# DreamWaterFound/self_commit_ORB-SLAM2

Measured on AMD Instinct MI355X. Metric: frames/s ORB extract+match (1000 feat, 640x480), higher is better.
Workload: dtype u8; 1 GPU; batch of 256 synthetic 640x480 frames per GPU (8 distinct resident batches per step, one launch set per batch), ORB extract (1000 feat, 8 levels, FAST 20/7) + brute-force Hamming SearchByBoW of consecutive frames; batch_per_gpu=256, streams=3, width=640, height=480, nfeatures=1000, parallelism=frames sharded, 1 rank(s), no data-path collective

## Files before the change

self_commit_orb-slam2_amd/csrc/orbx_kernels.hip:

```cpp
#include <algorithm>
#include "orbx_internal.h"

namespace {

struct OdTables {
    float pat[256][4];
    uint32_t disc[64][4];
};
constexpr int8_t kPattern[1024] = {
#include "orb_pattern.inc"
};
constexpr int kUmax[16] = {15, 15, 15, 15, 14, 14, 14, 13, 13, 12, 11, 10, 9, 8, 6, 3};
constexpr OdTables make_od_tables()
{
    OdTables t{};
    for (int i = 0; i < 256; i++) {
        t.pat[i][0] = (float)kPattern[4 * i]; t.pat[i][2] = (float)kPattern[4 * i + 1];
        t.pat[i][1] = (float)kPattern[4 * i + 2]; t.pat[i][3] = (float)kPattern[4 * i + 3];
    }
    for (int ml = 0; ml < 64; ml++)
        for (int j = 0; j < 4; j++) {
            const int mr = ml >> 1, mh = ml & 1;
            uint32_t m = 0u;
            if (mr < 31) {
// ... 746 lines not shown
        ncand = nToExpand + sh_misc[3];
        const bool finish = newN >= N || newN == prev;
        for (int j = tid; j < M; j += BT) {
            const int nd = (int)lab[j];
            if (!sel[nd]) { lab[j] = nmap[nd][0]; continue; }
            const uint32_t p = pts[j];
            const int nl = nmap[nd][ot_quadrant(p, box[cur][nd])];
            lab[j] = (uint32_t)nl;
            if (!finish && cnt[nxt][nl] > 1) atomicAdd(&qc[nxt][nl][ot_quadrant(p, box[nxt][nl])], 1u);
        }
        __syncthreads();
        if (tid == 0) { sh_misc[2] = 0; sh_misc[3] = 0; }
        nn = newN;
        cur = nxt;
        if (finish) break;
        if (!careful && nn + nToExpand * 3 > N) careful = true;
    }

    {
        uint32_t *best = &qc[cur ^ 1][0][0];
        OrbxLevelKp *out = lvlKp + (size_t)f * g->kpPerFrame + lv.kpBase;
        if (nn > lv.kpCap) { if (tid == 0) { atomicOr(stat, ORBX_DEV_ERR_KPCAP); atomicOr(statAll, ORBX_DEV_ERR_KPCAP); } nn = lv.kpCap; }
        __syncthreads();
        for (int i = tid; i < NODECAP; i += BT) best[i] = 0u;
        __syncthreads();
        for (int j = tid; j < M; j += BT) {
            const uint32_t nd = lab[j];
            if (nd < (uint32_t)NODECAP) atomicMax(&best[nd], (pts[j] & 0xff000000u) | (0x00ffffffu - (uint32_t)j));
        }
        __syncthreads();
        for (int i = tid; i < nn; i += BT) {
            const uint32_t b = pts[0x00ffffffu - (best[i] & 0x00ffffffu)];
            OrbxLevelKp kp;
            kp.x = (uint16_t)((b & 0xfff) + ORBX_BORDER); kp.y = (uint16_t)(((b >> 12) & 0xfff) + ORBX_BORDER);
            kp.score = (uint8_t)(b >> 24); kp.pad[0] = kp.pad[1] = kp.pad[2] = 0; kp.angle = 0.f; kp.ca = 1.f; kp.sb = 0.f;
            out[i] = kp;
        }
        if (tid == 0) lvlCnt[f * g->nlevels + l] = nn;
    }
}

__device__ __forceinline__ void host_pyramid_copy(const OrbxGeom *__restrict__ g, const OrbxCombMember *__restrict__ comb, const uint8_t *__restrict__ engPyr, int f, int chunk, int nchunks)
{
    uint4 *dst = (uint4 *)comb[f].hostPyr;
    if (!dst) return;
    const uint4 *src = (const uint4 *)(engPyr + (size_t)f * g->pyrBytes);
    const size_t n = g->pyrBytes >> 4, bt = blockDim.x, stride = (size_t)nchunks * bt;
    for (size_t i = (size_t)chunk * bt + threadIdx.x; i < n; i += stride) dst[i] = src[i];
}

template <int NODECAP>
__global__ __launch_bounds__(256) void k_octree(const OrbxGeom *__restrict__ g, const int *__restrict__ cellCount, const uint32_t *__restrict__ cellSlots,
                                                const uint8_t *__restrict__ binTab, uint32_t *__restrict__ ptBuf, uint32_t *__restrict__ labBuf,
                                                OrbxLevelKp *__restrict__ lvlKp, int *__restrict__ lvlCnt, int *__restrict__ status,
                                                const OrbxCombMember *__restrict__ comb, const uint8_t *__restrict__ engPyr, int *__restrict__ outBase)
{
    XCD_REMAP_XY(l, f);
    if (l >= g->nlevels) {
        host_pyramid_copy(g, comb, engPyr, f, l - g->nlevels, (int)gridDim.x - g->nlevels);
        return;
    }
    octree_body<NODECAP, 256>(g, cellCount, cellSlots, binTab, ptBuf, labBuf, lvlKp, lvlCnt, status, l, f, (int)gridDim.y);
    if (outBase && threadIdx.x == 0) {
        const int n = lvlCnt[f * g->nlevels + l];
        for (int j = l + 1; j < g->nlevels; j++) atomicAdd(&outBase[f * g->nlevels + j], n);
    }
}

__device__ __forceinline__ float sinf_poly_d(double x, double x2, int n, bool neg)
{
    const double c0 = 0x1p0, c1 = -0x1.ffffffd0c621cp-2, c2 = 0x1.55553e1068f19p-5, c3 = -0x1.6c087e89a359dp-10, c4 = 0x1.99343027bf8c3p-16;
    const double s1 = -0x1.555545995a603p-3, s2 = 0x1.1107605230bc4p-7, s3 = -0x1.994eb3774cf24p-13;
    if ((n & 1) == 0) {
        double x3 = x * x2, t1 = s2 + x2 * s3, x7 = x3 * x2, s = x + x3 * s1;
        return (float)(s + x7 * t1);
    } else {
        double k0 = neg ? -c0 : c0, k1 = neg ? -c1 : c1, k2 = neg ? -c2 : c2, k3 = neg ? -c3 : c3, k4 = neg ? -c4 : c4;
        double x4 = x2 * x2, u2 = k3 + x2 * k4, u1 = k0 + x2 * k1, x6 = x4 * x2, c = u1 + x4 * k2;
        return (float)(c + x6 * u2);
    }
}

__device__ __forceinline__ void sincosf_glibc(float y, float &sn, float &cs)
{
    double x = y;
    const uint32_t top = (__float_as_uint(y) >> 20) & 0x7ff;
    if (top < ((0x3f490fdbu >> 20) & 0x7ff)) {
        double x2 = x * x;
        if (top < ((0x39800000u >> 20) & 0x7ff)) { sn = y; cs = 1.0f; return; }
        sn = sinf_poly_d(x, x2, 0, false);
        cs = sinf_poly_d(x, x2, 1, false);
        return;
    }
    double r = x * 0x1.45F306DC9C883p+23;
    int n = ((int)r + 0x800000) >> 24;
    x = x - n * 0x1.921FB54442D18p0;
    const double sgn = ((n & 3) == 1 || (n & 3) == 2) ? -1.0 : 1.0;
    const bool neg = (n & 2) != 0;
    sn = sinf_poly_d(x * sgn, x * x, n, neg);
    cs = sinf_poly_d(x * sgn, x * x, n ^ 1, neg);
}

__device__ __forceinline__ float fast_atan2_deg(float y, float x)
{
    const float scale = (float)(180.0 / 3.14159265358979323846);
    const float p1 = 0.9997878412794807f * scale, p3 = -0.3258083974640975f * scale, p5 = 0.1555786518463281f * scale,
                p7 = -0.04432655554792128f * scale;
    float ax = fabsf(x), ay = fabsf(y), a, c, c2;
    if (ax >= ay) {
        c = ay / (ax + 2.220446049250313e-16f);
        c2 = c * c;
        a = (((p7 * c2 + p5) * c2 + p3) * c2 + p1) * c;
    } else {
        c = ax / (ay + 2.220446049250313e-16f);
        c2 = c * c;
        a = 90.f - (((p7 * c2 + p5) * c2 + p3) * c2 + p1) * c;
    }
    if (x < 0) a = 180.f - a;
    if (y < 0) a = 360.f - a;
    return a;
}

#define BT_W 64
#define BT_H 32
#define BT_P 80
#define BT_IH (BT_H + 6)

__device__ __forceinline__ int reflect101(int p, int len)
{
    if (p < 0) p = -p;
    if (p >= len) p = 2 * len - 2 - p;
    return p;
}

template <bool CLAMP>
__device__ __forceinline__ void blur_rows8(const OrbxGeom *__restrict__ g, const uint32_t *__restrict__ win, const int pitchW, uint32_t outw[8])
{
    const uint32_t k0 = g->taps[0], k1 = g->taps[1], k2 = g->taps[2], k3 = g->taps[3], k4 = g->taps[4], k5 = g->taps[5], k6 = g->taps[6];
    const uint32_t A0 = (k0 << 8) | (k1 << 16) | (k2 << 24), A1 = k3 | (k4 << 8) | (k5 << 16) | (k6 << 24);
    const uint32_t B0 = (k0 << 16) | (k1 << 24), B1 = k2 | (k3 << 8) | (k4 << 16) | (k5 << 24), B2 = k6;
    const uint32_t C0 = k0 << 24, C1 = k1 | (k2 << 8) | (k3 << 16) | (k4 << 24), C2 = k5 | (k6 << 8);
    const uint32_t D1 = k0 | (k1 << 8) | (k2 << 16) | (k3 << 24), D2 = k4 | (k5 << 8) | (k6 << 16);
    uint32_t hp[4][7];
#pragma unroll
    for (int m = 0; m < 7; m++) {
        uint32_t o[2][4];
#pragma unroll
        for (int s = 0; s < 2; s++) {
            const uint32_t *pw = win + (2 * m + s) * pitchW;
            const uint32_t w0 = pw[0], w1 = pw[1], w2 = pw[2];
            o[s][0] = __builtin_amdgcn_udot4(w1, A1, __builtin_amdgcn_udot4(w0, A0, 0u, false), false);
            o[s][1] = __builtin_amdgcn_udot4(w2, B2, __builtin_amdgcn_udot4(w1, B1, __builtin_amdgcn_udot4(w0, B0, 0u, false), false), false);
            o[s][2] = __builtin_amdgcn_udot4(w2, C2, __builtin_amdgcn_udot4(w1, C1, __builtin_amdgcn_udot4(w0, C0, 0u, false), false), false);
            o[s][3] = __builtin_amdgcn_udot4(w2, D2, __builtin_amdgcn_udot4(w1, D1, 0u, false), false);
        }
#pragma unroll
        for (int j = 0; j < 4; j++) hp[j][m] = o[0][j] | (o[1][j] << 16);
    }
    const uint32_t E0 = k0 | (k1 << 16), E1 = k2 | (k3 << 16), E2 = k4 | (k5 << 16), E3 = k6;
    const uint32_t O0 = k0 << 16, O1 = k1 | (k2 << 16), O2 = k3 | (k4 << 16), O3 = k5 | (k6 << 16);
#pragma unroll
    for (int q = 0; q < 8; q++) outw[q] = 0;
#pragma unroll
    for (int j = 0; j < 4; j++) {
        const uint32_t selo = j == 0 ? 0x03020106u : j == 1 ? 0x03020600u : j == 2 ? 0x03060100u : 0x06020100u;
#pragma unroll
        for (int q = 0; q < 8; q++) {
            const int t = q >> 1;
            const uint32_t sum = (q & 1) ? udot2(hp[j][t + 3], O3, udot2(hp[j][t + 2], O2, udot2(hp[j][t + 1], O1, udot2(hp[j][t], O0, 32768u))))
                                         : udot2(hp[j][t + 3], E3, udot2(hp[j][t + 2], E2, udot2(hp[j][t + 1], E1, udot2(hp[j][t], E0, 32768u))));
            if (CLAMP) outw[q] |= min(sum >> 16, 255u) << (8 * j);
            else outw[q] = __builtin_amdgcn_perm(sum, outw[q], selo);
        }
    }
}

template <bool CLAMP>
__device__ __forceinline__ void blur_body(const OrbxGeom *__restrict__ g, const uint8_t *__restrict__ img0, int img0Stride, size_t img0FramePitch,
                                          const uint8_t *__restrict__ pyr, uint8_t *__restrict__ blur, const int bx, const int f, uint32_t *__restrict__ in, const int lane,
                                          const bool store)
{
    int bases[ORBX_MAX_LEVELS];
    const int nl = g->nlevels;
    for (int i = 0; i < nl; i++) bases[i] = g->lv[i].blurTileBase;
    const int l = find_level(bases, nl, bx);
    const OrbxLevel &lv = g->lv[l];
    const int t = bx - lv.blurTileBase;
    const int X0 = (t % lv.blurTilesX) * BT_W, Y0 = (t / lv.blurTilesX) * BT_H;
    const int w = lv.w, h = lv.h;
    int pitch;
    const uint8_t *src = level_ptr(g, l, f, img0, img0Stride, img0FramePitch, pyr, pitch);
#pragma unroll
    for (int it = 0; it < 3; it++) {
        const int item = lane + 64 * it;
        if (item < BT_IH * 5) {
            const int r = (item * 205) >> 10, c = item - 5 * r;
            int y = reflect101(Y0 - 3 + r, h);
            y = min(max(y, 0), h - 1);
            const int x = X0 - 8 + 16 * c;
            const uint8_t *row = src + (size_t)y * pitch;
            uint4 v;
            if (x >= 0 && x + 15 < w) __builtin_memcpy(&v, row + x, 16);
            else {
                const int xs = min(max(x, 0), w - 16), d = x - xs;
                uint4 sv;
                __builtin_memcpy(&sv, row + xs, 16);
                if (d < 0) v = make_uint4(0u, 0u, sv.x, sv.y);
                else {
                    const uint32_t sw[8] = {sv.x, sv.y, sv.z, sv.w, 0u, 0u, 0u, 0u};
                    const int q = min(d >> 2, 4), bsh = d & 3;
                    uint32_t o[4];
#pragma unroll
                    for (int k = 0; k < 4; k++) {
                        uint32_t lo = 0u, hi = 0u;
#pragma unroll
                        for (int t = 0; t < 8; t++) { lo = (k + q == t) ? sw[t] : lo; hi = (k + q + 1 == t) ? sw[t] : hi; }
                        o[k] = bsh == 0 ? lo : bsh == 1 ? __builtin_amdgcn_alignbyte(hi, lo, 1) : bsh == 2 ? __builtin_amdgcn_alignbyte(hi, lo, 2) : __builtin_amdgcn_alignbyte(hi, lo, 3);
                    }
                    v = make_uint4(o[0], o[1], o[2], o[3]);
                }
            }
            *(uint4 *)(in + r * (BT_P / 4) + 4 * c) = v;
        }
    }
    __syncthreads();
    if (X0 == 0 || X0 + BT_W + 3 > w) {
        uint8_t *inb = (uint8_t *)in;
        if (lane < BT_IH) {
            uint8_t *rowb = inb + lane * BT_P;
            if (X0 == 0) { rowb[7] = rowb[9]; rowb[6] = rowb[10]; rowb[5] = rowb[11]; }
#pragma unroll
            for (int k = 0; k < 3; k++) {
                const int xo = w + k - X0 + 8, xi = w - 2 - k - X0 + 8;
                if (xo >= 0 && xo < BT_P && xi >= 0 && xi < BT_P) rowb[xo] = rowb[xi];
            }
        }
    }
    __syncthreads();
    const int gq = lane & 15, rg = lane >> 4;
    const int x = X0 + 4 * gq;
    if (!store || x >= w || Y0 + 8 * rg >= h) return;
    uint32_t outw[8];
    blur_rows8<CLAMP>(g, in + 8 * rg * (BT_P / 4) + gq + 1, BT_P / 4, outw);
    uint8_t *dst = blur + (size_t)f * g->pyrBytes + lv.off;
#pragma unroll
    for (int q = 0; q < 8; q++) {
        const int y = Y0 + 8 * rg + q;
        if (y >= h) break;
        *(uint32_t *)(dst + (size_t)y * lv.pitch + x) = outw[q];
    }
}

template <bool CLAMP>
__global__ __launch_bounds__(64) void k_blur(const OrbxGeom *__restrict__ g, const uint8_t *__restrict__ img0, int img0Stride, size_t img0FramePitch,
                                             const uint8_t *__restrict__ pyr, uint8_t *__restrict__ blur, const int *__restrict__ lvlCnt, int *__restrict__ outBase)
{
    __shared__ __attribute__((aligned(16))) uint32_t in[BT_IH * (BT_P / 4)];
    XCD_REMAP_XY(bx, f);
    if (bx == 0 && threadIdx.x == 0 && outBase) {
        int run = 0;
        for (int i = 0; i < g->nlevels; i++) { outBase[f * g->nlevels + i] = run; run += lvlCnt[f * g->nlevels + i]; }
    }
    blur_body<CLAMP>(g, img0, img0Stride, img0FramePitch, pyr, blur, bx, f, in, (int)threadIdx.x, true);
}

#define PB_THREADS 256
#define PB_ORG 16
#define PB_STAGE 4
__device__ __forceinline__ int pb_div(int item, uint32_t dv) { return (int)(__umul24((uint32_t)item, dv & 0xfffffu) >> (dv >> 20)); }
__device__ __forceinline__ uint32_t pb_mulhi24(uint32_t a, uint32_t b) { return __umulhi(a, b); }
template <bool EDGE>
__device__ __forceinline__ void pb_stage(uint8_t *__restrict__ bb, const uint8_t *__restrict__ src, const int sp, const int readable, const int w, const int h, const int P,
                                         const int s0, const int nr, const uint32_t divNc, const int tid)
{
    const int nc = (w + 15) >> 4, items = nr * nc;
    for (int i0 = 0; i0 < items; i0 += PB_THREADS * PB_STAGE) {
        uint4 v[PB_STAGE];
        int dOff[PB_STAGE];
#pragma unroll
        for (int k = 0; k < PB_STAGE; k++) {
            const int item = i0 + tid + k * PB_THREADS, it = min(item, items - 1);
            const int r = pb_div(it, divNc), c = it - (int)__umul24((uint32_t)r, (uint32_t)nc);
            int y = s0 - 3 + r;
            if (EDGE) {
                y = reflect101(y, h);
                y = min(max(y, 0), h - 1);
            }
            const uint8_t *row = src + (size_t)y * sp;
            const int x = 16 * c;
            if (x + 16 <= readable) __builtin_memcpy(&v[k], row + x, 16);
            else {
                uint32_t t[4] = {0u, 0u, 0u, 0u};
                for (int j = 0; x + j < w; j++) t[j >> 2] |= (uint32_t)row[x + j] << (8 * (j & 3));
                v[k] = make_uint4(t[0], t[1], t[2], t[3]);
            }
            dOff[k] = item < items ? (int)__umul24((uint32_t)r, (uint32_t)P) + PB_ORG + x : -1;
        }
#pragma unroll
        for (int k = 0; k < PB_STAGE; k++)
            if (dOff[k] >= 0) *(uint4 *)(bb + dOff[k]) = v[k];
    }
}

template <bool CLAMP>
__global__ __launch_bounds__(PB_THREADS) void k_pyr_band(const OrbxGeom *__restrict__ g, const int l, const uint8_t *__restrict__ img0, int img0Stride, size_t img0FramePitch,
                                                         const int readable, uint8_t *__restrict__ pyr, uint8_t *__restrict__ blur, const uint32_t *__restrict__ rsTab,
                                                         int *__restrict__ outBase)
{
    extern __shared__ __attribute__((aligned(16))) uint32_t band[];
    uint8_t *bb = (uint8_t *)band;
    XCD_REMAP_XY(b, f);
    const int nl = g->nlevels, tid = (int)threadIdx.x;
    if (l == 0 && b == 0 && tid < nl && outBase) outBase[f * nl + tid] = 0;
    const OrbxLevel &lv = g->lv[l];
    const int w = lv.w, h = lv.h, P = lv.bandPitch;
    const int s0 = b * lv.bandH, s1 = min(s0 + lv.bandH, h);
    const int nr = ((s1 - s0 + 7) & ~7) + 6;
    int sp;
    const uint8_t *src = level_ptr(g, l, f, img0, img0Stride, img0FramePitch, pyr, sp);
    if (s0 >= 3 && s0 - 3 + nr <= h) pb_stage<false>(bb, src, sp, readable, w, h, P, s0, nr, lv.bandDivNc, tid);
    else pb_stage<true>(bb, src, sp, readable, w, h, P, s0, nr, lv.bandDivNc, tid);
    __syncthreads();
    for (int r = tid; r < nr; r += PB_THREADS) {
        uint8_t *rowb = bb + r * P + PB_ORG;
        rowb[-1] = rowb[1]; rowb[-2] = rowb[2]; rowb[-3] = rowb[3];
#pragma unroll
        for (int k = 0; k < 3; k++) rowb[w + k] = rowb[w - 2 - k];
    }
    __syncthreads();
    {
        const int G4 = (w + 3) >> 2, items = G4 * ((s1 - s0 + 7) >> 3), PW = P >> 2;
        const uint32_t pitch = (uint32_t)lv.pitch;
        const bool full = ((s1 - s0) & 7) == 0;
        uint8_t *dst = blur + (size_t)f * g->pyrBytes + lv.off;
        for (int item = tid; item < items; item += PB_THREADS) {
            const int rgi = pb_div(item, lv.bandDivG4), gx = item - (int)__umul24((uint32_t)rgi, (uint32_t)G4);
            uint32_t outw[8];
            blur_rows8<CLAMP>(g, band + (int)__umul24((uint32_t)(8 * rgi), (uint32_t)PW) + gx + PB_ORG / 4 - 1, PW, outw);
            uint32_t o = (uint32_t)(s0 + 8 * rgi) * pitch + 4u * (uint32_t)gx;
            if (full) {
#pragma unroll
                for (int q = 0; q < 8; q++, o += pitch) *(uint32_t *)(dst + o) = outw[q];
            } else {
#pragma unroll
                for (int q = 0; q < 8; q++, o += pitch) {
                    if (s0 + 8 * rgi + q >= s1) break;
                    *(uint32_t *)(dst + o) = outw[q];
                }
            }
        }
    }
    if (l + 1 >= nl) return;
    const OrbxLevel &ln = g->lv[l + 1];
    const int d0 = (int)rsTab[lv.bandOff + b], d1 = (int)rsTab[lv.bandOff + b + 1];
    const int Gd = (ln.w + 3) >> 2, items = Gd * ((d1 - d0 + 7) >> 3);
    const uint32_t dpitch = (uint32_t)ln.pitch;
    const uint2 *rt = (const uint2 *)(rsTab + ln.rsRowOff);
    const uint32_t *ctab = rsTab + ln.rsColOff;
    uint8_t *dstBase = pyr + (size_t)f * g->pyrBytes + ln.off;
    const uint8_t *lrow0 = bb + PB_ORG - (s0 - 3) * P;
    for (int item = tid; item < items; item += PB_THREADS) {
        const int ch = pb_div(item, ln.bandDivG4), cg = item - (int)__umul24((uint32_t)ch, (uint32_t)Gd);
        const uint32_t *ct = ctab + 12u * (uint32_t)cg;
        const uint4 c0 = *(const uint4 *)ct, c1 = *(const uint4 *)(ct + 4), c2 = *(const uint4 *)(ct + 8);
        const int sx0 = (int)c0.x, sxa = sx0 & ~3;
        const uint32_t mis = (uint32_t)(sx0 & 3);
        const bool wide = (int)c0.y <= 7;
        const uint32_t sel[4] = {c0.z, c0.w, c1.x, c1.y}, coef[4] = {c1.z, c1.w, c2.x, c2.y};
        auto hpass = [&](int y, uint32_t hv[4]) {
            const uint8_t *row = lrow0 + (int)__umul24((uint32_t)y, (uint32_t)P);
            if (wide) {
                const uint32_t *p = (const uint32_t *)(row + sxa);
                const uint32_t a0 = p[0], a1 = p[1], a2 = p[2];
                const uint32_t v0 = __builtin_amdgcn_alignbyte(a1, a0, mis), v1 = __builtin_amdgcn_alignbyte(a2, a1, mis);
#pragma unroll
                for (int k = 0; k < 4; k++) hv[k] = udot2(__builtin_amdgcn_perm(v1, v0, sel[k]), coef[k], 0u) & 0x00fffff0u;
            } else {
                const uint8_t *S = row + sx0;
#pragma unroll
                for (int k = 0; k < 4; k++) {
                    const int off = (int)((c2.z >> (8 * k)) & 0xffu), off1 = (int)((c2.w >> (8 * k)) & 0xffu);
                    hv[k] = udot2((uint32_t)S[off] | ((uint32_t)S[off1] << 16), coef[k], 0u) & 0x00fffff0u;
                }
            }
        };
        uint32_t ha[4], hb[4];
        int ra = -1, rb = -1;
        const int dA = d0 + 8 * ch, nrow = min(8, d1 - dA);
        const uint2 *rtc = rt + (uint32_t)dA;
        uint2 tr[8];
#pragma unroll
        for (int r = 0; r < 8; r++) tr[r] = rtc[r];
        uint32_t o = (uint32_t)dA * dpitch + 4u * (uint32_t)cg;
#pragma unroll
        for (int r = 0; r < 8; r++, o += dpitch) {
            if (r >= nrow) break;
            const uint2 t = tr[r];
            const int y0 = (int)(t.x & 0xffffu), y1 = (int)(t.x >> 16);
            if (y0 != ra) {
                if (y0 == rb) {
#pragma unroll
                    for (int k = 0; k < 4; k++) ha[k] = hb[k];
                } else hpass(y0, ha);
                ra = y0;
            }
            if (y1 != rb) {
                if (y1 == ra) {
#pragma unroll
                    for (int k = 0; k < 4; k++) hb[k] = ha[k];
                } else hpass(y1, hb);
                rb = y1;
            }
            const uint32_t b0 = (t.y << 12) & 0x00fff000u, b1 = (t.y >> 4) & 0x00fff000u;
            uint32_t out = 0;
#pragma unroll
            for (int k = 0; k < 4; k++) out |= ((pb_mulhi24(b0, ha[k]) + pb_mulhi24(b1, hb[k]) + 2u) >> 2) << (8 * k);
            *(uint32_t *)(dstBase + o) = out;
        }
    }
}

#define OB_THREADS 1024
template <int NODECAP, bool CLAMP>
__global__ __launch_bounds__(OB_THREADS) void k_octree_blur(const OrbxGeom *__restrict__ g, const int *__restrict__ cellCount, const uint32_t *__restrict__ cellSlots,
                                                     const uint8_t *__restrict__ binTab, uint32_t *__restrict__ ptBuf, uint32_t *__restrict__ labBuf,
                                                     OrbxLevelKp *__restrict__ lvlKp, int *__restrict__ lvlCnt, int *__restrict__ status,
                                                     const OrbxCombMember *__restrict__ comb, const uint8_t *__restrict__ img0, int img0Stride, size_t img0FramePitch,
                                                     uint8_t *__restrict__ pyr, uint8_t *__restrict__ blur)
{
    extern __shared__ __attribute__((aligned(16))) uint32_t blurLds[];
    const int bx = (int)blockIdx.x, f = (int)blockIdx.y, nl = g->nlevels;
    if (bx < nl) { octree_body<NODECAP, OB_THREADS>(g, cellCount, cellSlots, binTab, ptBuf, labBuf, lvlKp, lvlCnt, status, bx, f, (int)gridDim.y); return; }
    if (bx < nl + ORBX_OCTREE_COPY_BLOCKS) { host_pyramid_copy(g, comb, pyr, f, bx - nl, ORBX_OCTREE_COPY_BLOCKS); return; }
    const int wv = (int)(threadIdx.x >> 6), tile = __builtin_amdgcn_readfirstlane((bx - nl - ORBX_OCTREE_COPY_BLOCKS) * (OB_THREADS / 64) + wv);
    blur_body<CLAMP>(g, img0, img0Stride, img0FramePitch, pyr, blur, min(tile, g->blurTiles - 1), f, blurLds + wv * (BT_IH * (BT_P / 4)), (int)(threadIdx.x & 63), tile < g->blurTiles);
}

__device__ __forceinline__ int wave_sum_dpp(int v)
{
    v += __builtin_amdgcn_update_dpp(0, v, 0xb1, 0xf, 0xf, true);
    v += __builtin_amdgcn_update_dpp(0, v, 0x4e, 0xf, 0xf, true);
    v += __builtin_amdgcn_update_dpp(0, v, 0x141, 0xf, 0xf, true);
    v += __builtin_amdgcn_update_dpp(0, v, 0x140, 0xf, 0xf, true);
    v += __builtin_amdgcn_update_dpp(0, v, 0x142, 0xa, 0xf, true);
    v += __builtin_amdgcn_update_dpp(0, v, 0x143, 0xc, 0xf, true);
    return __builtin_amdgcn_readlane(v, 63);
}

struct OdLevels {
    int nlevels, kpPerFrame, outCap, pad;
    unsigned long long pyrBytes;
    int kpBase[ORBX_MAX_LEVELS], off[ORBX_MAX_LEVELS], pitch[ORBX_MAX_LEVELS], patch[ORBX_MAX_LEVELS];
    float scale[ORBX_MAX_LEVELS];
};

#define OD_WPB 4
#define OD_R 18
#define OD_DW 10
#define OD_ROWS (2 * OD_R + 1)
#define OD_PATCH_DW (OD_ROWS * OD_DW)

__global__ __launch_bounds__(64 * OD_WPB) void k_orient_describe(const OdLevels A, const uint8_t *__restrict__ img0, int img0Stride, size_t img0FramePitch,
                                                                 const uint8_t *__restrict__ pyr, const uint8_t *__restrict__ blur, OrbxLevelKp *__restrict__ lvlKp,
                                                                 const int *__restrict__ lvlCnt, const int *__restrict__ outBase, orbx_keypoint *__restrict__ outKp,
                                                                 uint8_t *__restrict__ outDesc, int *__restrict__ outCnt, const int *__restrict__ status,
                                                                 int *__restrict__ outStatus)
{
    __shared__ uint32_t sPatch[OD_WPB][OD_PATCH_DW + 2];
    __shared__ __attribute__((aligned(16))) float sPat[256][4];
    __shared__ __attribute__((aligned(16))) uint32_t sDisc[64][4];
    __shared__ int sMom[OD_WPB][3];
    __shared__ int sBase[ORBX_MAX_LEVELS];
    __shared__ float sTrig[OD_WPB][3];
    XCD_REMAP_XY(bx, f);
    const int lane = threadIdx.x & 63;
    const int wv = __builtin_amdgcn_readfirstlane((int)(threadIdx.x >> 6));
    if (threadIdx.x < 256) {
        *(float4 *)sPat[threadIdx.x] = *(const float4 *)c_od.pat[threadIdx.x];
        ((uint32_t *)sDisc)[threadIdx.x] = ((const uint32_t *)c_od.disc)[threadIdx.x];
    }
    const int *cnts = lvlCnt + f * A.nlevels;
    if (!outBase && threadIdx.x < (unsigned)A.nlevels) {
        int run = 0;
        for (int i = 0; i < (int)threadIdx.x; i++) run += cnts[i];
        sBase[threadIdx.x] = run;
    }
    if (bx == 0 && threadIdx.x == 0) {
        int tot = 0;
        for (int i = 0; i < A.nlevels; i++) tot += cnts[i];
        outCnt[f] = tot;
        outStatus[f] = status[f];
        if (f == 0) outStatus[gridDim.y] = status[gridDim.y];
    }
    const int slot = bx * OD_WPB + wv;
    bool inRange = slot < A.kpPerFrame;
    int l = 0, kb = 0;
#pragma unroll
    for (int i = 1; i < ORBX_MAX_LEVELS; i++) {
        const bool ge = slot >= A.kpBase[i];
        l += ge ? 1 : 0; kb = ge ? A.kpBase[i] : kb;
    }
    const int idx = slot - kb;
    inRange = inRange && idx < cnts[l];
    const bool live = inRange;
    const uint2 kraw = *(const uint2 *)&lvlKp[(size_t)f * A.kpPerFrame + (inRange ? slot : 0)];
    const int kx = (int)(kraw.x & 0xffffu), ky = (int)(kraw.x >> 16);
    const int ksc = (int)(kraw.y & 0xffu);
    const int xa = (kx - OD_R) & ~3;
    int m10 = 0, m01 = 0;
    uint2 pw[3] = {make_uint2(0u, 0u), make_uint2(0u, 0u), make_uint2(0u, 0u)};
    uint4 wd = make_uint4(0u, 0u, 0u, 0u);
    const int r = lane >> 1, hf = lane & 1;
    if (inRange) {
        const int bp = A.pitch[l], up = l ? bp : img0Stride;
        const uint8_t *unb = l ? pyr + (size_t)f * A.pyrBytes + A.off[l] : img0 + (size_t)f * img0FramePitch;
        const uint8_t *bl = blur + (size_t)f * A.pyrBytes + A.off[l];
        if (r < 31) __builtin_memcpy(&wd, unb + (size_t)(ky + r - 15) * up + (kx - 15 + 16 * hf), 16);
#pragma unroll
        for (int t = 0; t < 3; t++) {
            const int item = lane + 64 * t;
            if (item < OD_ROWS * (OD_DW / 2)) {
                const int pr = (item * 205) >> 10, pc = item - (OD_DW / 2) * pr;
                __builtin_memcpy(&pw[t], bl + (size_t)(ky - OD_R + pr) * bp + xa + 8 * pc, 8);
            }
        }
    }
    __syncthreads();
    if (inRange && r < 31) {
        const uint4 mk = *(const uint4 *)sDisc[lane];
        const uint32_t wb = hf ? 0x10101010u : 0u;
        uint32_t s1 = 0u, sw = 0u;
        s1 = __builtin_amdgcn_udot4(wd.x & mk.x, 0x01010101u, s1, false); sw = __builtin_amdgcn_udot4(wd.x & mk.x, 0x03020100u + wb, sw, false);
        s1 = __builtin_amdgcn_udot4(wd.y & mk.y, 0x01010101u, s1, false); sw = __builtin_amdgcn_udot4(wd.y & mk.y, 0x07060504u + wb, sw, false);
        s1 = __builtin_amdgcn_udot4(wd.z & mk.z, 0x01010101u, s1, false); sw = __builtin_amdgcn_udot4(wd.z & mk.z, 0x0b0a0908u + wb, sw, false);
        s1 = __builtin_amdgcn_udot4(wd.w & mk.w, 0x01010101u, s1, false); sw = __builtin_amdgcn_udot4(wd.w & mk.w, 0x0f0e0d0cu + wb, sw, false);
        m10 = (int)sw - 15 * (int)s1;
        m01 = (r - 15) * (int)s1;
    }
    m10 = wave_sum_dpp(m10); m01 = wave_sum_dpp(m01);
    if (lane == 0) { sMom[wv][0] = m01; sMom[wv][1] = m10; sMom[wv][2] = live ? slot : -1; }
    if (live) {
#pragma unroll
        for (int t = 0; t < 3; t++) {
            const int item = lane + 64 * t;
            if (item < OD_ROWS * (OD_DW / 2)) *(uint2 *)&sPatch[wv][2 * item] = pw[t];
        }
    }
    __syncthreads();
    if (threadIdx.x < OD_WPB && sMom[threadIdx.x][2] >= 0) {
        const float ang = fast_atan2_deg((float)sMom[threadIdx.x][0], (float)sMom[threadIdx.x][1]);
        const float factorPI = (float)(3.1415926535897932384626433832795 / 180.f);
        float sn, cs;
        sincosf_glibc(ang * factorPI, sn, cs);
        sTrig[threadIdx.x][0] = cs; sTrig[threadIdx.x][1] = sn; sTrig[threadIdx.x][2] = ang;
        OrbxLevelKp *o = lvlKp + (size_t)f * A.kpPerFrame + sMom[threadIdx.x][2];
        o->angle = ang; o->ca = cs; o->sb = sn;
    }
    __syncthreads();
    if (!live) return;
    const float a = sTrig[wv][0], b = sTrig[wv][1];
    const uint8_t *pb = (const uint8_t *)sPatch[wv] + OD_R * (4 * OD_DW) + (kx - xa);
    unsigned long long bits[4];
    typedef float f2_t __attribute__((ext_vector_type(2)));
#pragma unroll
    for (int rd = 0; rd < 4; rd++) {
        const float4 pt = *(const float4 *)sPat[64 * rd + lane];
        const f2_t xs = {pt.x, pt.y}, ys = {pt.z, pt.w};
        const f2_t rr = xs * b + ys * a, cc = xs * a - ys * b;
        const int o0 = (int)__builtin_fmaf(__builtin_rintf(rr.x), (float)(4 * OD_DW), __builtin_rintf(cc.x));
        const int o1 = (int)__builtin_fmaf(__builtin_rintf(rr.y), (float)(4 * OD_DW), __builtin_rintf(cc.y));
        const int t0 = pb[o0], t1 = pb[o1];
        bits[rd] = __ballot(t0 < t1);
    }
    const int outIdx = (outBase ? outBase[f * A.nlevels + l] : sBase[l]) + idx;
    if (outIdx >= A.outCap) return;
    unsigned long long *d64 = (unsigned long long *)(outDesc + ((size_t)f * A.outCap + outIdx) * 32);
    if (lane < 4) d64[lane] = lane == 0 ? bits[0] : lane == 1 ? bits[1] : lane == 2 ? bits[2] : bits[3];
    if (lane == 0) {
        orbx_keypoint o;
        const float sc = A.scale[l];
        o.x = l ? (float)kx * sc : (float)kx;
        o.y = l ? (float)ky * sc : (float)ky;
        o.size = (float)A.patch[l]; o.angle = sTrig[wv][2]; o.response = (float)ksc; o.octave = l; o.class_id = -1;
        outKp[(size_t)f * A.outCap + outIdx] = o;
    }
}

__global__ __launch_bounds__(256) void k_comb_upload(const OrbxCombMember *__restrict__ tab, OrbxCombMember *__restrict__ tabCopy, uint8_t *__restrict__ staging, size_t framePitch)
{
    static_assert(sizeof(OrbxCombMember) % 8 == 0, "the table entry is copied in 8-byte words");
    if (blockIdx.x == 0 && threadIdx.x < sizeof(OrbxCombMember) / 8)
        ((unsigned long long *)&tabCopy[blockIdx.y])[threadIdx.x] = ((const unsigned long long *)&tab[blockIdx.y])[threadIdx.x];
    const uint4 *src = (const uint4 *)tab[blockIdx.y].srcImg;
    uint4 *dst = (uint4 *)(staging + (size_t)blockIdx.y * framePitch);
    const size_t n = framePitch >> 4, stride = (size_t)gridDim.x * 256;
    size_t i = (size_t)blockIdx.x * 256 + threadIdx.x;
    for (; i + 3 * stride < n; i += 4 * stride) {
        const uint4 a = src[i], b = src[i + stride], c = src[i + 2 * stride], d = src[i + 3 * stride];
        dst[i] = a; dst[i + stride] = b; dst[i + 2 * stride] = c; dst[i + 3 * stride] = d;
    }
    for (; i < n; i += stride) dst[i] = src[i];
}

__global__ __launch_bounds__(256) void k_comb_finish(const OrbxCombMember *__restrict__ tab, const int *__restrict__ engCnt, const int *__restrict__ engSt,
                                                     const orbx_keypoint *__restrict__ engKp, const uint8_t *__restrict__ engDesc, int cap, const uint8_t *__restrict__ engPyr,
                                                     size_t pyrBytes, const uint8_t *__restrict__ engImg, size_t framePitch, size_t kpOff, size_t descOff, int hostPyrHere,
                                                     unsigned *sync, unsigned long long *hostFlag)
{
    const int f = blockIdx.y;
    const OrbxCombMember m = tab[f];
    const int cnt = min(engCnt[f], cap);
    const size_t tid = (size_t)blockIdx.x * 256 + threadIdx.x, stride = (size_t)gridDim.x * 256;
    if (tid == 0) {
        const int st = engSt[f];
        int *d = (int *)m.devArena, *h = (int *)m.hostOut;
        d[0] = cnt; d[1] = st; d[2] = st;
        h[0] = cnt; h[1] = st; h[2] = st;
    }
    {
        const uint32_t *s = (const uint32_t *)(engKp + (size_t)f * cap);
        uint32_t *d = (uint32_t *)(m.devArena + kpOff), *h = (uint32_t *)(m.hostOut + kpOff);
        for (size_t i = tid; i < (size_t)cnt * 7; i += stride) { const uint32_t v = s[i]; d[i] = v; h[i] = v; }
    }
    {
        const uint4 *s = (const uint4 *)(engDesc + (size_t)f * cap * 32);
        uint4 *d = (uint4 *)(m.devArena + descOff), *h = (uint4 *)(m.hostOut + descOff);
        for (size_t i = tid; i < (size_t)cnt * 2; i += stride) { const uint4 v = s[i]; d[i] = v; h[i] = v; }
    }
    {
        const uint4 *s = (const uint4 *)(engPyr + (size_t)f * pyrBytes);
        uint4 *d = (uint4 *)m.devPyr, *h = hostPyrHere ? (uint4 *)m.hostPyr : nullptr;
        const size_t n = pyrBytes >> 4;
        if (h) for (size_t i = tid; i < n; i += stride) { const uint4 v = s[i]; d[i] = v; h[i] = v; }
        else for (size_t i = tid; i < n; i += stride) d[i] = s[i];
    }
    {
        const uint4 *s = (const uint4 *)(engImg + (size_t)f * framePitch);
        uint4 *d = (uint4 *)m.devImg;
        if (d) for (size_t i = tid; i < (framePitch >> 4); i += stride) d[i] = s[i];
    }
    if (hostFlag) {
        __syncthreads();
        if (threadIdx.x == 0) {
            __builtin_amdgcn_fence(__ATOMIC_RELEASE, "agent");
            if (__hip_atomic_fetch_add(sync, 1u, __ATOMIC_ACQ_REL, __HIP_MEMORY_SCOPE_AGENT) == gridDim.x * gridDim.y - 1) {
                __hip_atomic_store(sync, 0u, __ATOMIC_RELAXED, __HIP_MEMORY_SCOPE_AGENT);
                unsigned long long *cnt = (unsigned long long *)(sync + 2);
                const unsigned long long done = *cnt + 1;
                *cnt = done;
                __hip_atomic_store(hostFlag, done, __ATOMIC_RELEASE, __HIP_MEMORY_SCOPE_SYSTEM);
            }
        }
// ... 209 lines not shown
```

Baseline: 309,600 frames/s.

## March blur vertically per thread to reuse horizontal passes across row chunks

Replaces the per-item 8-row blur (which recomputed horizontal filter rows overlapping neighbouring chunks) with a per-thread vertical march that keeps a rolling window of horizontally filtered row pairs in registers, packed as 16-bit pairs and combined with udot2. Work is reassigned so each wavefront covers 64 column groups and lanes split the band's row chunks when there are fewer columns. This removes redundant horizontal tap work and the 6-row halo recomputation per chunk, at the cost of fewer independent work items (less parallelism per band) and more register pressure.

```diff
diff --git a/self_commit_orb-slam2_amd/csrc/orbx_kernels.hip b/self_commit_orb-slam2_amd/csrc/orbx_kernels.hip
--- a/self_commit_orb-slam2_amd/csrc/orbx_kernels.hip
+++ b/self_commit_orb-slam2_amd/csrc/orbx_kernels.hip
@@ -1072,6 +1072,55 @@
     }
 }
 
+template <bool CLAMP, bool FULL>
+__device__ __forceinline__ void blur_march(const OrbxGeom *__restrict__ g, const uint32_t *__restrict__ win, const int pitchW, const int nch, uint8_t *__restrict__ dst,
+                                           uint32_t o, const uint32_t pitch, const int rows)
+{
+    const uint32_t k0 = g->taps[0], k1 = g->taps[1], k2 = g->taps[2], k3 = g->taps[3], k4 = g->taps[4], k5 = g->taps[5], k6 = g->taps[6];
+    const uint32_t A0 = (k0 << 8) | (k1 << 16) | (k2 << 24), A1 = k3 | (k4 << 8) | (k5 << 16) | (k6 << 24);
+    const uint32_t B0 = (k0 << 16) | (k1 << 24), B1 = k2 | (k3 << 8) | (k4 << 16) | (k5 << 24), B2 = k6;
+    const uint32_t C0 = k0 << 24, C1 = k1 | (k2 << 8) | (k3 << 16) | (k4 << 24), C2 = k5 | (k6 << 8);
+    const uint32_t D1 = k0 | (k1 << 8) | (k2 << 16) | (k3 << 24), D2 = k4 | (k5 << 8) | (k6 << 16);
+    const uint32_t E0 = k0 | (k1 << 16), E1 = k2 | (k3 << 16), E2 = k4 | (k5 << 16), E3 = k6;
+    const uint32_t O0 = k0 << 16, O1 = k1 | (k2 << 16), O2 = k3 | (k4 << 16), O3 = k5 | (k6 << 16);
+    auto hpair = [&](const uint32_t *pw, uint32_t hp[4]) {
+        uint32_t h[2][4];
+#pragma unroll
+        for (int s = 0; s < 2; s++, pw += pitchW) {
+            const uint32_t w0 = pw[0], w1 = pw[1], w2 = pw[2];
+            h[s][0] = __builtin_amdgcn_udot4(w1, A1, __builtin_amdgcn_udot4(w0, A0, 0u, false), false);
+            h[s][1] = __builtin_amdgcn_udot4(w2, B2, __builtin_amdgcn_udot4(w1, B1, __builtin_amdgcn_udot4(w0, B0, 0u, false), false), false);
+            h[s][2] = __builtin_amdgcn_udot4(w2, C2, __builtin_amdgcn_udot4(w1, C1, __builtin_amdgcn_udot4(w0, C0, 0u, false), false), false);
+            h[s][3] = __builtin_amdgcn_udot4(w2, D2, __builtin_amdgcn_udot4(w1, D1, 0u, false), false);
+        }
+#pragma unroll
+        for (int j = 0; j < 4; j++) hp[j] = h[0][j] | (h[1][j] << 16);
+    };
+    uint32_t hp[4][4];
+    hpair(win, hp[0]);
+    hpair(win + 2 * pitchW, hp[1]);
+    hpair(win + 4 * pitchW, hp[2]);
+    win += 6 * pitchW;
+    for (int ch = 0; ch < nch; ch++) {
+#pragma unroll
+        for (int t = 0; t < 4; t++, win += 2 * pitchW, o += 2 * pitch) {
+            hpair(win, hp[(t + 3) & 3]);
+            const uint32_t *p0 = hp[t & 3], *p1 = hp[(t + 1) & 3], *p2 = hp[(t + 2) & 3], *p3 = hp[(t + 3) & 3];
+            uint32_t we = 0, wo = 0;
+#pragma unroll
+            for (int j = 0; j < 4; j++) {
+                const uint32_t selo = j == 0 ? 0x03020106u : j == 1 ? 0x03020600u : j == 2 ? 0x03060100u : 0x06020100u;
+                const uint32_t se = udot2(p3[j], E3, udot2(p2[j], E2, udot2(p1[j], E1, udot2(p0[j], E0, 32768u))));
+                const uint32_t so = udot2(p3[j], O3, udot2(p2[j], O2, udot2(p1[j], O1, udot2(p0[j], O0, 32768u))));
+                if (CLAMP) { we |= min(se >> 16, 255u) << (8 * j); wo |= min(so >> 16, 255u) << (8 * j); }
+                else { we = __builtin_amdgcn_perm(se, we, selo); wo = __builtin_amdgcn_perm(so, wo, selo); }
+            }
+            if (FULL || 8 * ch + 2 * t < rows) *(uint32_t *)(dst + o) = we;
+            if (FULL || 8 * ch + 2 * t + 1 < rows) *(uint32_t *)(dst + o + pitch) = wo;
+        }
+    }
+}
+
 template <bool CLAMP>
 __global__ __launch_bounds__(PB_THREADS) void k_pyr_band(const OrbxGeom *__restrict__ g, const int l, const uint8_t *__restrict__ img0, int img0Stride, size_t img0FramePitch,
                                                          const int readable, uint8_t *__restrict__ pyr, uint8_t *__restrict__ blur, const uint32_t *__restrict__ rsTab,
@@ -1099,25 +1148,21 @@
     }
     __syncthreads();
     {
-        const int G4 = (w + 3) >> 2, items = G4 * ((s1 - s0 + 7) >> 3), PW = P >> 2;
+        const int G4 = (w + 3) >> 2, C8 = (s1 - s0 + 7) >> 3, PW = P >> 2;
+        const int nFull = G4 >> 6, rem = G4 & 63, lane = tid & 63;
+        const int remSh = rem > 32 ? 6 : rem > 16 ? 5 : 4;
         const uint32_t pitch = (uint32_t)lv.pitch;
         const bool full = ((s1 - s0) & 7) == 0;
         uint8_t *dst = blur + (size_t)f * g->pyrBytes + lv.off;
-        for (int item = tid; item < items; item += PB_THREADS) {
-            const int rgi = pb_div(item, lv.bandDivG4), gx = item - (int)__umul24((uint32_t)rgi, (uint32_t)G4);
-            uint32_t outw[8];
-            blur_rows8<CLAMP>(g, band + (int)__umul24((uint32_t)(8 * rgi), (uint32_t)PW) + gx + PB_ORG / 4 - 1, PW, outw);
-            uint32_t o = (uint32_t)(s0 + 8 * rgi) * pitch + 4u * (uint32_t)gx;
-            if (full) {
-#pragma unroll
-                for (int q = 0; q < 8; q++, o += pitch) *(uint32_t *)(dst + o) = outw[q];
-            } else {
-#pragma unroll
-                for (int q = 0; q < 8; q++, o += pitch) {
-                    if (s0 + 8 * rgi + q >= s1) break;
-                    *(uint32_t *)(dst + o) = outw[q];
-                }
-            }
+        for (int wi = __builtin_amdgcn_readfirstlane(tid >> 6); wi < nFull + (rem != 0); wi += PB_THREADS / 64) {
+            const int sh = wi < nFull ? 6 : remSh;
+            const int c = (C8 + (64 >> sh) - 1) >> (6 - sh);
+            const int gx = 64 * wi + (lane & ((1 << sh) - 1)), ch0 = (lane >> sh) * c, nch = min(c, C8 - ch0);
+            if (gx >= G4 || nch <= 0) continue;
+            const uint32_t *win = band + (int)__umul24((uint32_t)(8 * ch0), (uint32_t)PW) + gx + PB_ORG / 4 - 1;
+            const uint32_t o = (uint32_t)(s0 + 8 * ch0) * pitch + 4u * (uint32_t)gx;
+            if (full) blur_march<CLAMP, true>(g, win, PW, nch, dst, o, pitch, 0);
+            else blur_march<CLAMP, false>(g, win, PW, nch, dst, o, pitch, s1 - s0 - 8 * ch0);
         }
     }
     if (l + 1 >= nl) return;
```

Result: no change. 311,300 frames/s, median of 6 (+0.5%).
